# rlorenzo/facet

Measured on NVIDIA B200. Metric: images/sec, higher is better.
Workload: dtype fp16

## Files before the change

facet_b200/csrc/attention_tc.cu:

```cuda
#include <cuda_bf16.h>

#include "common.cuh"
#include "kernels.h"
#include "tc_common.cuh"

namespace fb {

namespace {

constexpr int kTok = 257, kW = 1024, kD = 64;
constexpr int kThreadsAttn = 512;
constexpr float kScaleLog2 = 0.125f * 1.4426950408889634f;

constexpr int kOffQ = 0;
constexpr int kOffK = 32768;
constexpr int kOffV = 65536;
constexpr int kOffX = 98304;
constexpr int kWgBytes = 98304 + 8192;
constexpr int kSmemAttn = 2 * kWgBytes + 1024;

struct XArea {
    uint32_t q256h[32], k256h[32];
    float v256[64];
    float cls_p[264];
    float cls_red[16];
    float cls_o[64];
    float s256[2][128];
    float xmax[2][128];
    float xsum[2][128];
    uint64_t bar_qk, bar_v, bar_s, bar_pv;
};


__device__ __forceinline__ const uint4* sw_chunk(const uint8_t* tile, int r, int c) {
    return reinterpret_cast<const uint4*>(tile + r * 128 + ((c ^ (r & 7)) << 4));
}

template <bool F16>
__device__ __forceinline__ float mac2(uint32_t a, uint32_t b, float acc) {
    if (F16) {
        asm("{.reg .b16 al, ah, bl, bh;\n\t"
            "mov.b32 {al, ah}, %1;\n\t"
            "mov.b32 {bl, bh}, %2;\n\t"
            "fma.rn.f32.f16 %0, al, bl, %0;\n\t"
            "fma.rn.f32.f16 %0, ah, bh, %0;}"
            : "+f"(acc) : "r"(a), "r"(b));
        return acc;
    }
    acc = fmaf(tc::lo16<false>(a), tc::lo16<false>(b), acc);
    return fmaf(tc::hi16<false>(a), tc::hi16<false>(b), acc);
}
template <bool F16>
__device__ __forceinline__ void axpy2(float p, uint32_t p16, uint32_t v, float& a0, float& a1) {
    if (F16) {
        asm("{.reg .b16 pl, ph, vl, vh;\n\t"
            "mov.b32 {pl, ph}, %2;\n\t"
            "mov.b32 {vl, vh}, %3;\n\t"
            "fma.rn.f32.f16 %0, pl, vl, %0;\n\t"
            "fma.rn.f32.f16 %1, pl, vh, %1;}"
            : "+f"(a0), "+f"(a1) : "r"(p16), "r"(v));
        return;
    }
    a0 = fmaf(p, tc::lo16<false>(v), a0);
    a1 = fmaf(p, tc::hi16<false>(v), a1);
}

template <bool F16>
__device__ __forceinline__ float dot64_row(const uint8_t* tile, int r, const uint32_t* vec) {
    float acc = 0.f;
#pragma unroll
    for (int c = 0; c < 8; ++c) {
        const uint4 w = *sw_chunk(tile, r, c);
        const uint4 v = *reinterpret_cast<const uint4*>(vec + 4 * c);
        acc = mac2<F16>(w.x, v.x, acc);
        acc = mac2<F16>(w.y, v.y, acc);
        acc = mac2<F16>(w.z, v.z, acc);
        acc = mac2<F16>(w.w, v.w, acc);
    }
    return acc;
}

__device__ __forceinline__ uint64_t make_desc_mn_sw128(uint32_t smem_addr) {
    const uint32_t lo = ((smem_addr >> 4) & 0x3FFFu) | (64u << 16);
    const uint32_t hi = 64u | (1u << 14) | (2u << 29);
    return ((uint64_t)hi << 32) | lo;
}

__device__ __forceinline__ void umma_bf16_ts(uint32_t tmem_d, uint32_t tmem_a, uint64_t desc_b, uint32_t idesc, uint32_t accumulate) {
    asm volatile(
        "{\n\t.reg .pred p;\n\tsetp.ne.b32 p, %4, 0;\n\t"
        "tcgen05.mma.cta_group::1.kind::f16 [%0], [%1], %2, %3, p;\n\t}"
        ::"r"(tmem_d), "r"(tmem_a), "l"(desc_b), "r"(idesc), "r"(accumulate) : "memory");
}
__device__ __forceinline__ void tmem_st_32x16(uint32_t taddr, const uint32_t (&v)[16]) {
    asm volatile(
        "tcgen05.st.sync.aligned.32x32b.x16.b32 [%0], {%1,%2,%3,%4,%5,%6,%7,%8,%9,%10,%11,%12,%13,%14,%15,%16};"
        ::"r"(taddr), "r"(v[0]), "r"(v[1]), "r"(v[2]), "r"(v[3]), "r"(v[4]), "r"(v[5]), "r"(v[6]), "r"(v[7]), "r"(v[8]),
          "r"(v[9]), "r"(v[10]), "r"(v[11]), "r"(v[12]), "r"(v[13]), "r"(v[14]), "r"(v[15]) : "memory");
}
__device__ __forceinline__ void tmem_st_wait() { asm volatile("tcgen05.wait::st.sync.aligned;" ::: "memory"); }
__device__ __forceinline__ float ex2_fast(float x) {
    float y;
    asm("ex2.approx.ftz.f32 %0, %1;" : "=f"(y) : "f"(x));
    return y;
}
__device__ __forceinline__ void wg_sync(int wg) { asm volatile("bar.sync %0, 256;" ::"r"(wg + 1) : "memory"); }

template <bool F16>
__global__ void __launch_bounds__(kThreadsAttn, 1)
attention_tc_kernel(const __grid_constant__ CUtensorMap tmap_qkv, const uint16_t* __restrict__ qkv,
                    uint16_t* __restrict__ out, int n_pairs) {
    extern __shared__ uint8_t smem_raw[];
    __shared__ uint32_t tmem_slot;
    uint8_t* smem0 = smem_raw + ((1024u - ((uint32_t)__cvta_generic_to_shared(smem_raw) & 1023u)) & 1023u);
    const int tid = threadIdx.x, warp = tid >> 5, lane = tid & 31;
    const int wg = warp >> 3;
    const int wt = tid & 255;
    const int row = wt & 127;
    const int half = wt >> 7;
    uint8_t* smem = smem0 + wg * kWgBytes;
    XArea* X = reinterpret_cast<XArea*>(smem + kOffX);

    if (wt == 0) {
        tc::mbar_init(&X->bar_qk, 1);
        tc::mbar_init(&X->bar_v, 1);
        tc::mbar_init(&X->bar_s, 1);
        tc::mbar_init(&X->bar_pv, 1);
        tc::mbar_fence_init();
        tc::fence_proxy_async();
        if (tid == 0) tc::tma_prefetch_desc(&tmap_qkv);
    }
    if (warp == 0) tc::tmem_alloc(&tmem_slot, 512);
    tc::tc_fence_before();
    __syncthreads();
    tc::tc_fence_after();
    const uint32_t tmem = tmem_slot + wg * 256;
    const uint32_t lane_base = (uint32_t)(32 * (warp & 3)) << 16;
    const uint32_t t_s = tmem + lane_base + half * 128;
    const uint32_t t_p = tmem + lane_base + half * 128;
    const uint32_t t_o = tmem + lane_base + 64 + half * 32;
    const uint32_t idesc_s = tc::make_idesc16<F16>(128, 256);
    const uint32_t idesc_o = tc::make_idesc16<F16>(128, 64, 0, 1);

    const int first = blockIdx.x * 2 + wg, stride = gridDim.x * 2;
    auto issue_qk = [&](int pair) {
        const int b = pair >> 4, h = pair & 15, r0 = b * kTok;
        tc::mbar_expect_tx(&X->bar_qk, 4 * 16384);
        tc::tma_load_2d(&tmap_qkv, &X->bar_qk, smem + kOffQ, h * kD, r0);
        tc::tma_load_2d(&tmap_qkv, &X->bar_qk, smem + kOffQ + 16384, h * kD, r0 + 128);
        tc::tma_load_2d(&tmap_qkv, &X->bar_qk, smem + kOffK, kW + h * kD, r0);
        tc::tma_load_2d(&tmap_qkv, &X->bar_qk, smem + kOffK + 16384, kW + h * kD, r0 + 128);
    };
    auto issue_v = [&](int pair) {
        const int b = pair >> 4, h = pair & 15, r0 = b * kTok;
        tc::mbar_expect_tx(&X->bar_v, 2 * 16384);
        tc::tma_load_2d(&tmap_qkv, &X->bar_v, smem + kOffV, 2 * kW + h * kD, r0);
        tc::tma_load_2d(&tmap_qkv, &X->bar_v, smem + kOffV + 16384, 2 * kW + h * kD, r0 + 128);
    };
    if (wt == 0 && first < n_pairs) {
        issue_qk(first);
        issue_v(first);
    }

    auto load256 = [&](int pair) -> uint32_t {
        const int b = pair >> 4, h = pair & 15;
        return __ldg(reinterpret_cast<const uint32_t*>(qkv + ((size_t)b * kTok + 256) * (3 * kW) + (wt >> 5) * kW + h * kD + (wt & 31) * 2));
    };
    uint32_t pre256 = 0;
    if (wt < 96 && first < n_pairs) pre256 = load256(first);
    const int w8 = warp & 7;

    uint32_t ph_load = 0, ph_s = 0, ph_pv = 0;
    for (int pair = first; pair < n_pairs; pair += stride) {
        const int b = pair >> 4, h = pair & 15;
        const size_t tok0 = (size_t)b * kTok;
        const int next = pair + stride;
        if (wt < 96) {
            const int which = wt >> 5, i2 = wt & 31;
            if (which == 0) X->q256h[i2] = pre256;
            else if (which == 1) X->k256h[i2] = pre256;
            else {
                X->v256[2 * i2] = tc::lo16<F16>(pre256);
                X->v256[2 * i2 + 1] = tc::hi16<F16>(pre256);
            }
        }
        wg_sync(wg);
        tc::mbar_wait(&X->bar_qk, ph_load);
        if (wt == 0) {
            const uint64_t dk = tc::make_desc_k_sw128(tc::smem_u32(smem + kOffK));
            const uint64_t dq = tc::make_desc_k_sw128(tc::smem_u32(smem + kOffQ));
#pragma unroll
            for (int k = 0; k < 4; ++k) tc::umma_bf16(tmem, dq + 2 * k, dk + 2 * k, idesc_s, k != 0);
            tc::umma_commit(&X->bar_s);
        }
        X->s256[half][row] = dot64_row<F16>(smem + kOffQ + half * 16384, row, X->k256h);

#pragma unroll 1
        for (int t = 0; t < 2; ++t) {
            tc::mbar_wait(&X->bar_s, ph_s);
            ph_s ^= 1;
            tc::tc_fence_after();
            if (t == 1 && wt == 0 && next < n_pairs) issue_qk(next);
            float mx;
            {
                uint32_t va[32], vb[32];
                float m0 = half == 0 ? X->s256[t][row] : -INFINITY, m1 = -INFINITY, m2 = -INFINITY, m3 = -INFINITY;
                tc::tmem_ld_32x32(t_s, va);
#pragma unroll 1
                for (int c = 0; c < 4; c += 2) {
                    tc::tmem_ld_wait();
                    tc::tmem_ld_32x32(t_s + (c + 1) * 32, vb);
#pragma unroll
                    for (int j = 0; j < 32; j += 4) {
                        m0 = fmaxf(m0, __uint_as_float(va[j]));
                        m1 = fmaxf(m1, __uint_as_float(va[j + 1]));
                        m2 = fmaxf(m2, __uint_as_float(va[j + 2]));
                        m3 = fmaxf(m3, __uint_as_float(va[j + 3]));
                    }
                    tc::tmem_ld_wait();
                    if (c + 2 < 4) tc::tmem_ld_32x32(t_s + (c + 2) * 32, va);
#pragma unroll
                    for (int j = 0; j < 32; j += 4) {
                        m0 = fmaxf(m0, __uint_as_float(vb[j]));
                        m1 = fmaxf(m1, __uint_as_float(vb[j + 1]));
                        m2 = fmaxf(m2, __uint_as_float(vb[j + 2]));
                        m3 = fmaxf(m3, __uint_as_float(vb[j + 3]));
                    }
                }
                mx = fmaxf(fmaxf(m0, m1), fmaxf(m2, m3));
            }
            X->xmax[half][row] = mx;
            wg_sync(wg);
            mx = fmaxf(X->xmax[0][row], X->xmax[1][row]);
            const float s256 = X->s256[t][row];
            const float mxs = mx * kScaleLog2;
            const float p_last = ex2_fast(fmaf(s256, kScaleLog2, -mxs));
            float sum0 = half == 0 ? p_last : 0.f, sum1 = 0.f;
            {
                uint32_t va[32], vb[32];
                auto emit = [&](const uint32_t (&v)[32], int c) {
                    uint32_t pk[16];
#pragma unroll
                    for (int j = 0; j < 16; ++j) {
                        const float x0 = fmaf(__uint_as_float(v[2 * j]), kScaleLog2, -mxs);
                        const float x1 = fmaf(__uint_as_float(v[2 * j + 1]), kScaleLog2, -mxs);
                        const float p0 = ex2_fast(x0), p1 = ex2_fast(x1);
                        sum0 += p0;
                        sum1 += p1;
                        pk[j] = tc::pack16<F16>(p0, p1);
                    }
                    tmem_st_32x16(t_p + c * 16, pk);
                };
                tc::tmem_ld_32x32(t_s, va);
#pragma unroll 1
                for (int c = 0; c < 4; c += 2) {
                    tc::tmem_ld_wait();
                    tc::tmem_ld_32x32(t_s + (c + 1) * 32, vb);
                    emit(va, c);
                    tc::tmem_ld_wait();
                    if (c + 2 < 4) tc::tmem_ld_32x32(t_s + (c + 2) * 32, va);
                    emit(vb, c + 1);
                }
            }
            X->xsum[half][row] = sum0 + sum1;
            tmem_st_wait();
            tc::tc_fence_before();
            wg_sync(wg);
            const float inv_l = 1.0f / (X->xsum[0][row] + X->xsum[1][row]);
            if (t == 0) tc::mbar_wait(&X->bar_v, ph_load);
            if (wt == 0) {
                tc::tc_fence_after();
                const uint32_t vbase = tc::smem_u32(smem + kOffV);
#pragma unroll
                for (int i = 0; i < 16; ++i)
                    umma_bf16_ts(tmem + 64, tmem + (i < 8 ? 8 * i : 128 + 8 * (i - 8)), make_desc_mn_sw128(vbase + i * 2048), idesc_o, i != 0);
                tc::umma_commit(&X->bar_pv);
            }
            if (t == 0) {
                const float sa = dot64_row<F16>(smem + kOffK, wt, X->q256h);
                float s_last = -INFINITY;
                if (wt == 0) {
                    s_last = 0.f;
#pragma unroll
                    for (int d = 0; d < 32; ++d) s_last = mac2<F16>(X->q256h[d], X->k256h[d], s_last);
                }
                float cm = fmaxf(sa, s_last);
#pragma unroll
                for (int o = 16; o > 0; o >>= 1) cm = fmaxf(cm, __shfl_xor_sync(0xffffffffu, cm, o));
                if (lane == 0) X->cls_red[w8] = cm;
                wg_sync(wg);
                cm = fmaxf(fmaxf(fmaxf(X->cls_red[0], X->cls_red[1]), fmaxf(X->cls_red[2], X->cls_red[3])),
                           fmaxf(fmaxf(X->cls_red[4], X->cls_red[5]), fmaxf(X->cls_red[6], X->cls_red[7])));
                const float pa = ex2_fast((sa - cm) * kScaleLog2);
                X->cls_p[wt] = pa;
                float sum = pa;
                if (wt == 0) {
                    const float pl = ex2_fast((s_last - cm) * kScaleLog2);
                    X->cls_p[256] = pl;
                    sum += pl;
                }
#pragma unroll
                for (int o = 16; o > 0; o >>= 1) sum += __shfl_xor_sync(0xffffffffu, sum, o);
                if (lane == 0) X->cls_red[8 + w8] = sum;
            } else {
                if (wt < 96 && next < n_pairs) pre256 = load256(next);
                float a8[8];
#pragma unroll
                for (int k = 0; k < 8; ++k) a8[k] = 0.f;
#pragma unroll
                for (int i = 0; i < 8; ++i) {
                    const int key = lane + 32 * i;
                    const uint4 q = *sw_chunk(smem + kOffV, key, w8);
                    const float pj = X->cls_p[key];
                    const uint32_t p16 = F16 ? tc::pack_f16(pj, pj) : 0u;
                    axpy2<F16>(pj, p16, q.x, a8[0], a8[1]);
                    axpy2<F16>(pj, p16, q.y, a8[2], a8[3]);
                    axpy2<F16>(pj, p16, q.z, a8[4], a8[5]);
                    axpy2<F16>(pj, p16, q.w, a8[6], a8[7]);
                }
                float b4[4], b2[2];
                const bool u16 = (lane & 16) != 0, u8 = (lane & 8) != 0, u4 = (lane & 4) != 0;
#pragma unroll
                for (int k = 0; k < 4; ++k) {
                    const float send = u16 ? a8[k] : a8[k + 4];
                    const float keep = u16 ? a8[k + 4] : a8[k];
                    b4[k] = keep + __shfl_xor_sync(0xffffffffu, send, 16);
                }
#pragma unroll
                for (int k = 0; k < 2; ++k) {
                    const float send = u8 ? b4[k] : b4[k + 2];
                    const float keep = u8 ? b4[k + 2] : b4[k];
                    b2[k] = keep + __shfl_xor_sync(0xffffffffu, send, 8);
                }
                float tot1 = (u4 ? b2[1] : b2[0]) + __shfl_xor_sync(0xffffffffu, u4 ? b2[0] : b2[1], 4);
                tot1 += __shfl_xor_sync(0xffffffffu, tot1, 2);
                tot1 += __shfl_xor_sync(0xffffffffu, tot1, 1);
                if ((lane & 3) == 0) X->cls_o[8 * w8 + (u16 ? 4 : 0) + (u8 ? 2 : 0) + (u4 ? 1 : 0)] = tot1;
            }
            tc::mbar_wait(&X->bar_pv, ph_pv);
            ph_pv ^= 1;
            tc::tc_fence_after();
            {
                uint32_t v0[32];
                tc::tmem_ld_32x32(t_o, v0);
                tc::tmem_ld_wait();
                tc::tc_fence_before();
                wg_sync(wg);
                if (t == 0 && wt == 0) {
                    tc::tc_fence_after();
                    const uint64_t dk = tc::make_desc_k_sw128(tc::smem_u32(smem + kOffK));
                    const uint64_t dq = tc::make_desc_k_sw128(tc::smem_u32(smem + kOffQ + 16384));
#pragma unroll
                    for (int k = 0; k < 4; ++k) tc::umma_bf16(tmem, dq + 2 * k, dk + 2 * k, idesc_s, k != 0);
                    tc::umma_commit(&X->bar_s);
                }
                if (t == 1) {
                    if (wt == 0 && next < n_pairs) issue_v(next);
                    if (wt < 64) {
                        const float tot = ((X->cls_red[8] + X->cls_red[9]) + (X->cls_red[10] + X->cls_red[11])) +
                                          ((X->cls_red[12] + X->cls_red[13]) + (X->cls_red[14] + X->cls_red[15]));
                        const float o = X->cls_o[wt] + X->cls_p[256] * X->v256[wt];
                        out[(tok0 + 256) * kW + h * kD + wt] = (uint16_t)(tc::pack16<F16>(o / tot, 0.f) & 0xffffu);
                    }
                }
                uint4* dst = reinterpret_cast<uint4*>(out + (tok0 + t * 128 + row) * kW + h * kD + half * 32);
#pragma unroll
                for (int q = 0; q < 4; ++q) {
                    float o[8];
#pragma unroll
                    for (int j = 0; j < 8; ++j) {
                        const int dcol = 8 * q + j;
                        o[j] = (__uint_as_float(v0[dcol]) + p_last * X->v256[half * 32 + dcol]) * inv_l;
                    }
                    dst[q] = make_uint4(tc::pack16<F16>(o[0], o[1]), tc::pack16<F16>(o[2], o[3]), tc::pack16<F16>(o[4], o[5]),
                                        tc::pack16<F16>(o[6], o[7]));
                }
            }
        }
        ph_load ^= 1;
        wg_sync(wg);
    }
    tc::tc_fence_before();
    __syncthreads();
    tc::tc_fence_after();
    if (warp == 0) tc::tmem_dealloc(tmem_slot, 512);
}

}

int launch_attention_tc(const void* d_qkv, int batch, void* d_out, int f16, cudaStream_t stream) {
    FB_REQUIRE(d_qkv && d_out && batch >= 1, "fb_vit_attention: bad arguments");
    CUtensorMap tm;
    int rc = make_tmap_bf16_2d(&tm, d_qkv, (uint64_t)batch * kTok, 3 * kW, 3 * kW, 128, 64);
    if (rc) return rc;
    static PerDeviceFlag attr_set;
    if (!attr_set.get()) {
        FB_CUDA_OK(cudaFuncSetAttribute(attention_tc_kernel<false>, cudaFuncAttributeMaxDynamicSharedMemorySize, kSmemAttn));
        FB_CUDA_OK(cudaFuncSetAttribute(attention_tc_kernel<true>, cudaFuncAttributeMaxDynamicSharedMemorySize, kSmemAttn));
        attr_set.set();
    }
    const int n_pairs = batch * 16;
    int grid = (n_pairs + 1) / 2;
    if (grid > sm_count()) grid = sm_count();
    if (f16) attention_tc_kernel<true><<<grid, kThreadsAttn, kSmemAttn, stream>>>(tm, reinterpret_cast<const uint16_t*>(d_qkv),
                                                                              reinterpret_cast<uint16_t*>(d_out), n_pairs);
    else attention_tc_kernel<false><<<grid, kThreadsAttn, kSmemAttn, stream>>>(tm, reinterpret_cast<const uint16_t*>(d_qkv),
                                                                            reinterpret_cast<uint16_t*>(d_out), n_pairs);
    FB_CUDA_OK(cudaGetLastError());
    return 0;
}

}
```

facet_b200/csrc/tc_common.cuh:

```cuda
#pragma once
#include <cuda.h>
#include <cuda_bf16.h>
#include <cuda_fp16.h>
#include <cuda_runtime.h>
#include <stdint.h>

namespace fb {
namespace tc {

__device__ __forceinline__ uint32_t smem_u32(const void* p) { return (uint32_t)__cvta_generic_to_shared(p); }

__device__ __forceinline__ bool elect_one() {
    uint32_t pred = 0;
    asm volatile(
        "{\n\t.reg .pred P;\n\telect.sync _|P, 0xffffffff;\n\tselp.b32 %0, 1, 0, P;\n\t}"
        : "=r"(pred));
    return pred != 0;
}

__device__ __forceinline__ void mbar_init(uint64_t* bar, uint32_t count) {
    asm volatile("mbarrier.init.shared::cta.b64 [%0], %1;" ::"r"(smem_u32(bar)), "r"(count));
}
__device__ __forceinline__ void mbar_fence_init() {
    asm volatile("fence.mbarrier_init.release.cluster;" ::: "memory");
}
__device__ __forceinline__ void fence_proxy_async() {
    asm volatile("fence.proxy.async.shared::cta;" ::: "memory");
}
__device__ __forceinline__ void mbar_expect_tx(uint64_t* bar, uint32_t bytes) {
    asm volatile("mbarrier.arrive.expect_tx.shared::cta.b64 _, [%0], %1;" ::"r"(smem_u32(bar)), "r"(bytes) : "memory");
}
__device__ __forceinline__ void mbar_arrive(uint64_t* bar) {
    asm volatile("mbarrier.arrive.shared::cta.b64 _, [%0];" ::"r"(smem_u32(bar)) : "memory");
}
__device__ __forceinline__ void mbar_wait(uint64_t* bar, uint32_t parity) {
    const uint32_t addr = smem_u32(bar);
    asm volatile(
        "{\n\t"
        ".reg .pred P1;\n\t"
        "WAIT_%=:\n\t"
        "mbarrier.try_wait.parity.shared::cta.b64 P1, [%0], %1;\n\t"
        "@P1 bra DONE_%=;\n\t"
        "bra WAIT_%=;\n\t"
        "DONE_%=:\n\t"
        "}" ::"r"(addr), "r"(parity) : "memory");
}

__device__ __forceinline__ void tma_prefetch_desc(const CUtensorMap* m) {
    asm volatile("prefetch.tensormap [%0];" ::"l"(reinterpret_cast<uint64_t>(m)) : "memory");
}
__device__ __forceinline__ void tma_load_2d(const CUtensorMap* m, uint64_t* bar, void* smem_dst, int c0, int c1) {
    asm volatile(
        "cp.async.bulk.tensor.2d.shared::cluster.global.mbarrier::complete_tx::bytes [%0], [%1, {%3, %4}], [%2];"
        ::"r"(smem_u32(smem_dst)), "l"(reinterpret_cast<uint64_t>(m)), "r"(smem_u32(bar)), "r"(c0), "r"(c1)
        : "memory");
}

__device__ __forceinline__ void tma_load_2d_multicast(const CUtensorMap* m, uint64_t* bar, void* smem_dst, int c0, int c1,
                                                      uint16_t cta_mask) {
    asm volatile(
        "cp.async.bulk.tensor.2d.shared::cluster.global.mbarrier::complete_tx::bytes.multicast::cluster [%0], [%1, {%3, %4}], [%2], %5;"
        ::"r"(smem_u32(smem_dst)), "l"(reinterpret_cast<uint64_t>(m)), "r"(smem_u32(bar)), "r"(c0), "r"(c1), "h"(cta_mask)
        : "memory");
}
__device__ __forceinline__ uint32_t mapa_u32(uint32_t local, uint32_t rank) {
    uint32_t r;
    asm volatile("mapa.shared::cluster.u32 %0, %1, %2;" : "=r"(r) : "r"(local), "r"(rank));
    return r;
}
__device__ __forceinline__ void mbar_expect_tx_cluster(uint32_t cluster_addr, uint32_t bytes) {
    asm volatile("mbarrier.arrive.expect_tx.shared::cluster.b64 _, [%0], %1;" ::"r"(cluster_addr), "r"(bytes) : "memory");
}
__device__ __forceinline__ void mbar_arrive_cluster(uint32_t cluster_addr) {
    asm volatile("mbarrier.arrive.shared::cluster.b64 _, [%0];" ::"r"(cluster_addr) : "memory");
}
__device__ __forceinline__ void tma_load_2d_pair(const CUtensorMap* m, uint32_t bar_cluster_addr, void* smem_dst, int c0, int c1) {
    asm volatile(
        "cp.async.bulk.tensor.2d.cta_group::2.shared::cluster.global.mbarrier::complete_tx::bytes [%0], [%1, {%3, %4}], [%2];"
        ::"r"(smem_u32(smem_dst)), "l"(reinterpret_cast<uint64_t>(m)), "r"(bar_cluster_addr), "r"(c0), "r"(c1)
        : "memory");
}
__device__ __forceinline__ void tmem_alloc_pair(uint32_t* smem_dst, uint32_t cols) {
    asm volatile("tcgen05.alloc.cta_group::2.sync.aligned.shared::cta.b32 [%0], %1;" ::"r"(smem_u32(smem_dst)), "r"(cols) : "memory");
    asm volatile("tcgen05.relinquish_alloc_permit.cta_group::2.sync.aligned;" ::: "memory");
}
__device__ __forceinline__ void tmem_dealloc_pair(uint32_t taddr, uint32_t cols) {
    asm volatile("tcgen05.dealloc.cta_group::2.sync.aligned.b32 %0, %1;" ::"r"(taddr), "r"(cols) : "memory");
}
__device__ __forceinline__ void umma_bf16_pair(uint32_t tmem_d, uint64_t desc_a, uint64_t desc_b, uint32_t idesc, uint32_t accumulate) {
    asm volatile(
        "{\n\t.reg .pred p;\n\tsetp.ne.b32 p, %4, 0;\n\t"
        "tcgen05.mma.cta_group::2.kind::f16 [%0], %1, %2, %3, p;\n\t}"
        ::"r"(tmem_d), "l"(desc_a), "l"(desc_b), "r"(idesc), "r"(accumulate) : "memory");
}
__device__ __forceinline__ void umma_commit_pair(uint64_t* bar, uint16_t cta_mask) {
    asm volatile("tcgen05.commit.cta_group::2.mbarrier::arrive::one.shared::cluster.multicast::cluster.b64 [%0], %1;"
                 ::"r"(smem_u32(bar)), "h"(cta_mask) : "memory");
}
__device__ __forceinline__ uint32_t cluster_ctarank() {
    uint32_t r;
    asm volatile("mov.u32 %0, %%cluster_ctarank;" : "=r"(r));
    return r;
}
__device__ __forceinline__ void cluster_sync_all() {
    asm volatile("barrier.cluster.arrive.release.aligned;\n\tbarrier.cluster.wait.acquire.aligned;" ::: "memory");
}

__device__ __forceinline__ void tmem_alloc(uint32_t* smem_dst, uint32_t cols) {
    asm volatile("tcgen05.alloc.cta_group::1.sync.aligned.shared::cta.b32 [%0], %1;" ::"r"(smem_u32(smem_dst)), "r"(cols) : "memory");
    asm volatile("tcgen05.relinquish_alloc_permit.cta_group::1.sync.aligned;" ::: "memory");
}
__device__ __forceinline__ void tmem_dealloc(uint32_t taddr, uint32_t cols) {
    asm volatile("tcgen05.dealloc.cta_group::1.sync.aligned.b32 %0, %1;" ::"r"(taddr), "r"(cols) : "memory");
}
__device__ __forceinline__ void tc_fence_before() { asm volatile("tcgen05.fence::before_thread_sync;" ::: "memory"); }
__device__ __forceinline__ void tc_fence_after() { asm volatile("tcgen05.fence::after_thread_sync;" ::: "memory"); }

__device__ __forceinline__ void umma_bf16(uint32_t tmem_d, uint64_t desc_a, uint64_t desc_b, uint32_t idesc, uint32_t accumulate) {
    asm volatile(
        "{\n\t.reg .pred p;\n\tsetp.ne.b32 p, %4, 0;\n\t"
        "tcgen05.mma.cta_group::1.kind::f16 [%0], %1, %2, %3, p;\n\t}"
        ::"r"(tmem_d), "l"(desc_a), "l"(desc_b), "r"(idesc), "r"(accumulate) : "memory");
}
__device__ __forceinline__ void umma_commit(uint64_t* bar) {
    asm volatile("tcgen05.commit.cta_group::1.mbarrier::arrive::one.shared::cluster.b64 [%0];" ::"r"(smem_u32(bar)) : "memory");
}

__device__ __forceinline__ void umma_commit_multicast(uint64_t* bar, uint16_t cta_mask) {
    asm volatile("tcgen05.commit.cta_group::1.mbarrier::arrive::one.shared::cluster.multicast::cluster.b64 [%0], %1;"
                 ::"r"(smem_u32(bar)), "h"(cta_mask) : "memory");
}

__host__ __device__ constexpr uint32_t make_idesc_bf16(int m, int n, int a_mn_major = 0, int b_mn_major = 0) {
    return (1u << 4) | (1u << 7) | (1u << 10) | ((uint32_t)a_mn_major << 15) | ((uint32_t)b_mn_major << 16) |
           ((uint32_t)(n >> 3) << 17) | ((uint32_t)(m >> 4) << 24);
}
__host__ __device__ constexpr uint32_t make_idesc_f16(int m, int n, int a_mn_major = 0, int b_mn_major = 0) {
    return (1u << 4) | ((uint32_t)a_mn_major << 15) | ((uint32_t)b_mn_major << 16) |
           ((uint32_t)(n >> 3) << 17) | ((uint32_t)(m >> 4) << 24);
}
template <bool F16>
__host__ __device__ constexpr uint32_t make_idesc16(int m, int n, int a_mn_major = 0, int b_mn_major = 0) {
    return F16 ? make_idesc_f16(m, n, a_mn_major, b_mn_major) : make_idesc_bf16(m, n, a_mn_major, b_mn_major);
}

__device__ __forceinline__ uint64_t make_desc_k_sw128(uint32_t smem_addr) {
    const uint32_t lo = ((smem_addr >> 4) & 0x3FFFu) | (1u << 16);
    const uint32_t hi = 64u | (1u << 14) | (2u << 29);
    return ((uint64_t)hi << 32) | lo;
}

__device__ __forceinline__ void tmem_ld_32x32(uint32_t taddr, uint32_t (&v)[32]) {
    asm volatile(
        "tcgen05.ld.sync.aligned.32x32b.x32.b32 "
        "{%0,%1,%2,%3,%4,%5,%6,%7,%8,%9,%10,%11,%12,%13,%14,%15,%16,%17,%18,%19,%20,%21,%22,%23,%24,%25,%26,%27,%28,%29,%30,%31}, [%32];"
        : "=r"(v[0]), "=r"(v[1]), "=r"(v[2]), "=r"(v[3]), "=r"(v[4]), "=r"(v[5]), "=r"(v[6]), "=r"(v[7]), "=r"(v[8]),
          "=r"(v[9]), "=r"(v[10]), "=r"(v[11]), "=r"(v[12]), "=r"(v[13]), "=r"(v[14]), "=r"(v[15]), "=r"(v[16]),
          "=r"(v[17]), "=r"(v[18]), "=r"(v[19]), "=r"(v[20]), "=r"(v[21]), "=r"(v[22]), "=r"(v[23]), "=r"(v[24]),
          "=r"(v[25]), "=r"(v[26]), "=r"(v[27]), "=r"(v[28]), "=r"(v[29]), "=r"(v[30]), "=r"(v[31])
        : "r"(taddr) : "memory");
}
__device__ __forceinline__ void tmem_ld_wait() { asm volatile("tcgen05.wait::ld.sync.aligned;" ::: "memory"); }

__device__ __forceinline__ uint32_t pack_bf16(float a, float b) {
    __nv_bfloat162 v = __floats2bfloat162_rn(a, b);
    return *reinterpret_cast<uint32_t*>(&v);
}
__device__ __forceinline__ uint32_t pack_f16(float a, float b) {
    __half2 v = __floats2half2_rn(a, b);
    return *reinterpret_cast<uint32_t*>(&v);
}
template <bool F16>
__device__ __forceinline__ uint32_t pack16(float a, float b) { return F16 ? pack_f16(a, b) : pack_bf16(a, b); }
template <bool F16>
__device__ __forceinline__ float lo16(uint32_t w) {
    if (F16) return __half2float(__ushort_as_half((unsigned short)(w & 0xffffu)));
    return __uint_as_float(w << 16);
}
template <bool F16>
__device__ __forceinline__ float hi16(uint32_t w) {
    if (F16) return __half2float(__ushort_as_half((unsigned short)(w >> 16)));
    return __uint_as_float(w & 0xffff0000u);
}

}

int make_tmap_bf16_2d(CUtensorMap* out, const void* base, uint64_t rows, uint64_t cols, uint64_t row_stride_elems,
                      uint32_t box_rows, uint32_t box_cols);

}
```

Measured before the change: 4183.

## Warp-specialize attention kernel with double-buffered TMA pipeline and TMA output stores

Restructures the ViT attention kernel from two independent 256-thread workgroups into a warp-specialized design: one TMA producer warp, one MMA issuer warp, eight softmax warps and two warps dedicated to the CLS token row. Inputs are double-buffered with full/empty mbarriers, and the score matrix is split into four 128-key blocks whose partial softmaxes are merged with rescaling. Outputs are staged in shared memory and written with TMA stores, and the dot product uses four independent accumulators. The aim is to overlap loads, MMA and softmax across pairs, at the cost of more complex synchronization and one pair per CTA instead of two.

```diff
diff --git a/facet_b200/csrc/attention_tc.cu b/facet_b200/csrc/attention_tc.cu
--- a/facet_b200/csrc/attention_tc.cu
+++ b/facet_b200/csrc/attention_tc.cu
@@ -9,28 +9,29 @@
 namespace {
 
 constexpr int kTok = 257, kW = 1024, kD = 64;
-constexpr int kThreadsAttn = 512;
+constexpr int kThreadsAttn = 384;
 constexpr float kScaleLog2 = 0.125f * 1.4426950408889634f;
 
 constexpr int kOffQ = 0;
 constexpr int kOffK = 32768;
 constexpr int kOffV = 65536;
-constexpr int kOffX = 98304;
-constexpr int kWgBytes = 98304 + 8192;
-constexpr int kSmemAttn = 2 * kWgBytes + 1024;
-
-struct XArea {
-    uint32_t q256h[32], k256h[32];
-    float v256[64];
+constexpr int kBufBytes = 98304;
+constexpr int kTileBytes = 16384;
+
+struct Tok256 {
+    uint32_t q[32], k[32];
+    float v[64];
+};
+struct Ctl {
+    Tok256 tok[2];
     float cls_p[264];
-    float cls_red[16];
+    float cls_red[4];
     float cls_o[64];
-    float s256[2][128];
-    float xmax[2][128];
-    float xsum[2][128];
-    uint64_t bar_qk, bar_v, bar_s, bar_pv;
+    uint64_t full[2], empty[2];
+    uint64_t s_ready[4], p_ready[4], o_ready[4], blk_free[4];
 };
-
+constexpr int kSmemAttn = 2 * kBufBytes + (int)sizeof(Ctl) + 1024;
+constexpr uint32_t kEmptyArrivals = 256 + 64 + 1;
 
 __device__ __forceinline__ const uint4* sw_chunk(const uint8_t* tile, int r, int c) {
     return reinterpret_cast<const uint4*>(tile + r * 128 + ((c ^ (r & 7)) << 4));
@@ -67,17 +68,17 @@
 
 template <bool F16>
 __device__ __forceinline__ float dot64_row(const uint8_t* tile, int r, const uint32_t* vec) {
-    float acc = 0.f;
+    float a0 = 0.f, a1 = 0.f, a2 = 0.f, a3 = 0.f;
 #pragma unroll
     for (int c = 0; c < 8; ++c) {
         const uint4 w = *sw_chunk(tile, r, c);
         const uint4 v = *reinterpret_cast<const uint4*>(vec + 4 * c);
-        acc = mac2<F16>(w.x, v.x, acc);
-        acc = mac2<F16>(w.y, v.y, acc);
-        acc = mac2<F16>(w.z, v.z, acc);
-        acc = mac2<F16>(w.w, v.w, acc);
-    }
-    return acc;
+        a0 = mac2<F16>(w.x, v.x, a0);
+        a1 = mac2<F16>(w.y, v.y, a1);
+        a2 = mac2<F16>(w.z, v.z, a2);
+        a3 = mac2<F16>(w.w, v.w, a3);
+    }
+    return (a0 + a1) + (a2 + a3);
 }
 
 __device__ __forceinline__ uint64_t make_desc_mn_sw128(uint32_t smem_addr) {
@@ -104,286 +105,278 @@
     asm("ex2.approx.ftz.f32 %0, %1;" : "=f"(y) : "f"(x));
     return y;
 }
-__device__ __forceinline__ void wg_sync(int wg) { asm volatile("bar.sync %0, 256;" ::"r"(wg + 1) : "memory"); }
+__device__ __forceinline__ void cls_sync() { asm volatile("bar.sync 1, 64;" ::: "memory"); }
 
 template <bool F16>
 __global__ void __launch_bounds__(kThreadsAttn, 1)
-attention_tc_kernel(const __grid_constant__ CUtensorMap tmap_qkv, const uint16_t* __restrict__ qkv,
-                    uint16_t* __restrict__ out, int n_pairs) {
+attention_tc_kernel(const __grid_constant__ CUtensorMap tmap_qkv, const __grid_constant__ CUtensorMap tmap_out,
+                    const uint16_t* __restrict__ qkv, uint16_t* __restrict__ out, int n_pairs) {
     extern __shared__ uint8_t smem_raw[];
     __shared__ uint32_t tmem_slot;
-    uint8_t* smem0 = smem_raw + ((1024u - ((uint32_t)__cvta_generic_to_shared(smem_raw) & 1023u)) & 1023u);
+    uint8_t* smem = smem_raw + ((1024u - ((uint32_t)__cvta_generic_to_shared(smem_raw) & 1023u)) & 1023u);
+    Ctl* C = reinterpret_cast<Ctl*>(smem + 2 * kBufBytes);
     const int tid = threadIdx.x, warp = tid >> 5, lane = tid & 31;
-    const int wg = warp >> 3;
-    const int wt = tid & 255;
-    const int row = wt & 127;
-    const int half = wt >> 7;
-    uint8_t* smem = smem0 + wg * kWgBytes;
-    XArea* X = reinterpret_cast<XArea*>(smem + kOffX);
-
-    if (wt == 0) {
-        tc::mbar_init(&X->bar_qk, 1);
-        tc::mbar_init(&X->bar_v, 1);
-        tc::mbar_init(&X->bar_s, 1);
-        tc::mbar_init(&X->bar_pv, 1);
+
+    if (tid == 0) {
+        for (int b = 0; b < 2; ++b) {
+            tc::mbar_init(&C->full[b], 2);
+            tc::mbar_init(&C->empty[b], kEmptyArrivals);
+        }
+        for (int k = 0; k < 4; ++k) {
+            tc::mbar_init(&C->s_ready[k], 1);
+            tc::mbar_init(&C->p_ready[k], 128);
+            tc::mbar_init(&C->o_ready[k], 1);
+            tc::mbar_init(&C->blk_free[k], 128);
+        }
         tc::mbar_fence_init();
         tc::fence_proxy_async();
-        if (tid == 0) tc::tma_prefetch_desc(&tmap_qkv);
+        tc::tma_prefetch_desc(&tmap_qkv);
+        tc::tma_prefetch_desc(&tmap_out);
     }
     if (warp == 0) tc::tmem_alloc(&tmem_slot, 512);
     tc::tc_fence_before();
     __syncthreads();
     tc::tc_fence_after();
-    const uint32_t tmem = tmem_slot + wg * 256;
-    const uint32_t lane_base = (uint32_t)(32 * (warp & 3)) << 16;
-    const uint32_t t_s = tmem + lane_base + half * 128;
-    const uint32_t t_p = tmem + lane_base + half * 128;
-    const uint32_t t_o = tmem + lane_base + 64 + half * 32;
-    const uint32_t idesc_s = tc::make_idesc16<F16>(128, 256);
-    const uint32_t idesc_o = tc::make_idesc16<F16>(128, 64, 0, 1);
-
-    const int first = blockIdx.x * 2 + wg, stride = gridDim.x * 2;
-    auto issue_qk = [&](int pair) {
-        const int b = pair >> 4, h = pair & 15, r0 = b * kTok;
-        tc::mbar_expect_tx(&X->bar_qk, 4 * 16384);
-        tc::tma_load_2d(&tmap_qkv, &X->bar_qk, smem + kOffQ, h * kD, r0);
-        tc::tma_load_2d(&tmap_qkv, &X->bar_qk, smem + kOffQ + 16384, h * kD, r0 + 128);
-        tc::tma_load_2d(&tmap_qkv, &X->bar_qk, smem + kOffK, kW + h * kD, r0);
-        tc::tma_load_2d(&tmap_qkv, &X->bar_qk, smem + kOffK + 16384, kW + h * kD, r0 + 128);
-    };
-    auto issue_v = [&](int pair) {
-        const int b = pair >> 4, h = pair & 15, r0 = b * kTok;
-        tc::mbar_expect_tx(&X->bar_v, 2 * 16384);
-        tc::tma_load_2d(&tmap_qkv, &X->bar_v, smem + kOffV, 2 * kW + h * kD, r0);
-        tc::tma_load_2d(&tmap_qkv, &X->bar_v, smem + kOffV + 16384, 2 * kW + h * kD, r0 + 128);
-    };
-    if (wt == 0 && first < n_pairs) {
-        issue_qk(first);
-        issue_v(first);
-    }
-
-    auto load256 = [&](int pair) -> uint32_t {
-        const int b = pair >> 4, h = pair & 15;
-        return __ldg(reinterpret_cast<const uint32_t*>(qkv + ((size_t)b * kTok + 256) * (3 * kW) + (wt >> 5) * kW + h * kD + (wt & 31) * 2));
-    };
-    uint32_t pre256 = 0;
-    if (wt < 96 && first < n_pairs) pre256 = load256(first);
-    const int w8 = warp & 7;
-
-    uint32_t ph_load = 0, ph_s = 0, ph_pv = 0;
-    for (int pair = first; pair < n_pairs; pair += stride) {
-        const int b = pair >> 4, h = pair & 15;
-        const size_t tok0 = (size_t)b * kTok;
-        const int next = pair + stride;
-        if (wt < 96) {
-            const int which = wt >> 5, i2 = wt & 31;
-            if (which == 0) X->q256h[i2] = pre256;
-            else if (which == 1) X->k256h[i2] = pre256;
-            else {
-                X->v256[2 * i2] = tc::lo16<F16>(pre256);
-                X->v256[2 * i2 + 1] = tc::hi16<F16>(pre256);
-            }
-        }
-        wg_sync(wg);
-        tc::mbar_wait(&X->bar_qk, ph_load);
-        if (wt == 0) {
-            const uint64_t dk = tc::make_desc_k_sw128(tc::smem_u32(smem + kOffK));
-            const uint64_t dq = tc::make_desc_k_sw128(tc::smem_u32(smem + kOffQ));
-#pragma unroll
-            for (int k = 0; k < 4; ++k) tc::umma_bf16(tmem, dq + 2 * k, dk + 2 * k, idesc_s, k != 0);
-            tc::umma_commit(&X->bar_s);
-        }
-        X->s256[half][row] = dot64_row<F16>(smem + kOffQ + half * 16384, row, X->k256h);
-
-#pragma unroll 1
-        for (int t = 0; t < 2; ++t) {
-            tc::mbar_wait(&X->bar_s, ph_s);
-            ph_s ^= 1;
+    const uint32_t tmem = tmem_slot;
+
+    if (warp < 8) {
+        const int t = warp >> 2;
+        const int row = 32 * (warp & 3) + lane;
+        const uint32_t t_row = tmem + ((uint32_t)(32 * (warp & 3)) << 16);
+        auto block_softmax = [&](int blk, uint32_t ph, float& m_out, float& l_out) {
+            const uint32_t ta = t_row + 128 * blk;
+            tc::mbar_wait(&C->s_ready[blk], ph);
             tc::tc_fence_after();
-            if (t == 1 && wt == 0 && next < n_pairs) issue_qk(next);
-            float mx;
-            {
-                uint32_t va[32], vb[32];
-                float m0 = half == 0 ? X->s256[t][row] : -INFINITY, m1 = -INFINITY, m2 = -INFINITY, m3 = -INFINITY;
-                tc::tmem_ld_32x32(t_s, va);
-#pragma unroll 1
-                for (int c = 0; c < 4; c += 2) {
-                    tc::tmem_ld_wait();
-                    tc::tmem_ld_32x32(t_s + (c + 1) * 32, vb);
-#pragma unroll
-                    for (int j = 0; j < 32; j += 4) {
-                        m0 = fmaxf(m0, __uint_as_float(va[j]));
-                        m1 = fmaxf(m1, __uint_as_float(va[j + 1]));
-                        m2 = fmaxf(m2, __uint_as_float(va[j + 2]));
-                        m3 = fmaxf(m3, __uint_as_float(va[j + 3]));
-                    }
-                    tc::tmem_ld_wait();
-                    if (c + 2 < 4) tc::tmem_ld_32x32(t_s + (c + 2) * 32, va);
-#pragma unroll
-                    for (int j = 0; j < 32; j += 4) {
-                        m0 = fmaxf(m0, __uint_as_float(vb[j]));
-                        m1 = fmaxf(m1, __uint_as_float(vb[j + 1]));
-                        m2 = fmaxf(m2, __uint_as_float(vb[j + 2]));
-                        m3 = fmaxf(m3, __uint_as_float(vb[j + 3]));
-                    }
-                }
-                mx = fmaxf(fmaxf(m0, m1), fmaxf(m2, m3));
-            }
-            X->xmax[half][row] = mx;
-            wg_sync(wg);
-            mx = fmaxf(X->xmax[0][row], X->xmax[1][row]);
-            const float s256 = X->s256[t][row];
+            uint32_t v[4][32];
+#pragma unroll
+            for (int c = 0; c < 4; ++c) tc::tmem_ld_32x32(ta + 32 * c, v[c]);
+            tc::tmem_ld_wait();
+            float m0 = -INFINITY, m1 = -INFINITY, m2 = -INFINITY, m3 = -INFINITY;
+#pragma unroll
+            for (int c = 0; c < 4; ++c)
+#pragma unroll
+                for (int j = 0; j < 32; j += 4) {
+                    m0 = fmaxf(m0, __uint_as_float(v[c][j]));
+                    m1 = fmaxf(m1, __uint_as_float(v[c][j + 1]));
+                    m2 = fmaxf(m2, __uint_as_float(v[c][j + 2]));
+                    m3 = fmaxf(m3, __uint_as_float(v[c][j + 3]));
+                }
+            const float mx = fmaxf(fmaxf(m0, m1), fmaxf(m2, m3));
             const float mxs = mx * kScaleLog2;
-            const float p_last = ex2_fast(fmaf(s256, kScaleLog2, -mxs));
-            float sum0 = half == 0 ? p_last : 0.f, sum1 = 0.f;
-            {
-                uint32_t va[32], vb[32];
-                auto emit = [&](const uint32_t (&v)[32], int c) {
-                    uint32_t pk[16];
-#pragma unroll
-                    for (int j = 0; j < 16; ++j) {
-                        const float x0 = fmaf(__uint_as_float(v[2 * j]), kScaleLog2, -mxs);
-                        const float x1 = fmaf(__uint_as_float(v[2 * j + 1]), kScaleLog2, -mxs);
-                        const float p0 = ex2_fast(x0), p1 = ex2_fast(x1);
-                        sum0 += p0;
-                        sum1 += p1;
-                        pk[j] = tc::pack16<F16>(p0, p1);
-                    }
-                    tmem_st_32x16(t_p + c * 16, pk);
-                };
-                tc::tmem_ld_32x32(t_s, va);
-#pragma unroll 1
-                for (int c = 0; c < 4; c += 2) {
-                    tc::tmem_ld_wait();
-                    tc::tmem_ld_32x32(t_s + (c + 1) * 32, vb);
-                    emit(va, c);
-                    tc::tmem_ld_wait();
-                    if (c + 2 < 4) tc::tmem_ld_32x32(t_s + (c + 2) * 32, va);
-                    emit(vb, c + 1);
-                }
-            }
-            X->xsum[half][row] = sum0 + sum1;
+            float sum0 = 0.f, sum1 = 0.f;
+#pragma unroll
+            for (int c = 0; c < 4; ++c) {
+                uint32_t pk[16];
+#pragma unroll
+                for (int j = 0; j < 16; ++j) {
+                    const float p0 = ex2_fast(fmaf(__uint_as_float(v[c][2 * j]), kScaleLog2, -mxs));
+                    const float p1 = ex2_fast(fmaf(__uint_as_float(v[c][2 * j + 1]), kScaleLog2, -mxs));
+                    sum0 += p0;
+                    sum1 += p1;
+                    pk[j] = tc::pack16<F16>(p0, p1);
+                }
+                tmem_st_32x16(ta + 16 * c, pk);
+            }
             tmem_st_wait();
             tc::tc_fence_before();
-            wg_sync(wg);
-            const float inv_l = 1.0f / (X->xsum[0][row] + X->xsum[1][row]);
-            if (t == 0) tc::mbar_wait(&X->bar_v, ph_load);
-            if (wt == 0) {
+            tc::mbar_arrive(&C->p_ready[blk]);
+            m_out = mx;
+            l_out = sum0 + sum1;
+        };
+        int it = 0;
+        for (int pair = blockIdx.x; pair < n_pairs; pair += gridDim.x, ++it) {
+            const int b = it & 1;
+            const uint32_t ph = it & 1;
+            uint8_t* buf = smem + b * kBufBytes;
+            const Tok256& tk = C->tok[b];
+            tc::mbar_wait(&C->full[b], (it >> 1) & 1);
+            float m0, l0, m1, l1;
+            block_softmax(2 * t, ph, m0, l0);
+            block_softmax(2 * t + 1, ph, m1, l1);
+            uint32_t o0[2][32];
+            tc::mbar_wait(&C->o_ready[2 * t], ph);
+            tc::tc_fence_after();
+            tc::tmem_ld_32x32(t_row + 128 * (2 * t) + 64, o0[0]);
+            tc::tmem_ld_32x32(t_row + 128 * (2 * t) + 96, o0[1]);
+            tc::tmem_ld_wait();
+            tc::tc_fence_before();
+            tc::mbar_arrive(&C->blk_free[2 * t]);
+            const float s_last = dot64_row<F16>(buf + kOffQ + t * kTileBytes, row, tk.k);
+            const float m = fmaxf(fmaxf(m0, m1), s_last);
+            const float a0 = ex2_fast((m0 - m) * kScaleLog2), a1 = ex2_fast((m1 - m) * kScaleLog2);
+            const float a2 = ex2_fast((s_last - m) * kScaleLog2);
+            const float inv_l = 1.0f / (fmaf(a0, l0, a1 * l1) + a2);
+            const float c0 = a0 * inv_l, c1 = a1 * inv_l, cl = a2 * inv_l;
+
+            tc::mbar_wait(&C->o_ready[2 * t + 1], ph);
+            tc::tc_fence_after();
+            uint8_t* stage = buf + kOffQ + t * kTileBytes;
+#pragma unroll
+            for (int c = 0; c < 2; ++c) {
+                uint32_t u1[32];
+                tc::tmem_ld_32x32(t_row + 128 * (2 * t + 1) + 64 + 32 * c, u1);
+                tc::tmem_ld_wait();
+                if (c == 1) {
+                    tc::tc_fence_before();
+                    tc::mbar_arrive(&C->blk_free[2 * t + 1]);
+                }
+#pragma unroll
+                for (int q = 0; q < 4; ++q) {
+                    uint32_t w[4];
+#pragma unroll
+                    for (int k = 0; k < 4; ++k) {
+                        const int d = 8 * q + 2 * k;
+                        const float2 vv = *reinterpret_cast<const float2*>(&tk.v[32 * c + d]);
+                        const float o0a = fmaf(__uint_as_float(u1[d]), c1, fmaf(__uint_as_float(o0[c][d]), c0, cl * vv.x));
+                        const float o0b = fmaf(__uint_as_float(u1[d + 1]), c1, fmaf(__uint_as_float(o0[c][d + 1]), c0, cl * vv.y));
+                        w[k] = tc::pack16<F16>(o0a, o0b);
+                    }
+                    *reinterpret_cast<uint4*>(stage + row * 128 + (((4 * c + q) ^ (row & 7)) << 4)) = make_uint4(w[0], w[1], w[2], w[3]);
+                }
+            }
+            tc::fence_proxy_async();
+            if (t == 0) asm volatile("bar.sync 2, 128;" ::: "memory");
+            else asm volatile("bar.sync 3, 128;" ::: "memory");
+            if (row == 0) {
+                tc::tma_store_2d(&tmap_out, stage, (pair & 15) * kD, (pair >> 4) * kTok + t * 128);
+                tc::bulk_commit_group();
+                tc::bulk_wait_group_read0();
+            }
+            tc::mbar_arrive(&C->empty[b]);
+        }
+        if (row == 0) tc::bulk_wait_group0();
+    } else if (warp == 8) {
+        int it = 0;
+        for (int pair = blockIdx.x; pair < n_pairs; pair += gridDim.x, ++it) {
+            const int b = it & 1;
+            if (it >= 2) tc::mbar_wait(&C->empty[b], ((it >> 1) - 1) & 1);
+            const int img = pair >> 4, h = pair & 15, r0 = img * kTok;
+            uint8_t* buf = smem + b * kBufBytes;
+            if (lane == 0) {
+                tc::mbar_expect_tx(&C->full[b], 6 * kTileBytes);
+                tc::tma_load_2d(&tmap_qkv, &C->full[b], buf + kOffQ, h * kD, r0);
+                tc::tma_load_2d(&tmap_qkv, &C->full[b], buf + kOffQ + kTileBytes, h * kD, r0 + 128);
+                tc::tma_load_2d(&tmap_qkv, &C->full[b], buf + kOffK, kW + h * kD, r0);
+                tc::tma_load_2d(&tmap_qkv, &C->full[b], buf + kOffK + kTileBytes, kW + h * kD, r0 + 128);
+                tc::tma_load_2d(&tmap_qkv, &C->full[b], buf + kOffV, 2 * kW + h * kD, r0);
+                tc::tma_load_2d(&tmap_qkv, &C->full[b], buf + kOffV + kTileBytes, 2 * kW + h * kD, r0 + 128);
+            }
+            const uint32_t* src = reinterpret_cast<const uint32_t*>(qkv + ((size_t)r0 + 256) * (3 * kW) + h * kD) + lane;
+            const uint32_t q = __ldg(src), k = __ldg(src + kW / 2), v = __ldg(src + kW);
+            C->tok[b].q[lane] = q;
+            C->tok[b].k[lane] = k;
+            C->tok[b].v[2 * lane] = tc::lo16<F16>(v);
+            C->tok[b].v[2 * lane + 1] = tc::hi16<F16>(v);
+            __syncwarp();
+            if (lane == 0) tc::mbar_arrive(&C->full[b]);
+        }
+    } else if (warp == 9) {
+        if (lane == 0) {
+            const uint32_t idesc_s = tc::make_idesc16<F16>(128, 128);
+            const uint32_t idesc_o = tc::make_idesc16<F16>(128, 64, 0, 1);
+            int it = 0;
+            for (int pair = blockIdx.x; pair < n_pairs; pair += gridDim.x, ++it) {
+                const int b = it & 1;
+                const uint32_t ph = it & 1;
+                const uint8_t* buf = smem + b * kBufBytes;
+                tc::mbar_wait(&C->full[b], (it >> 1) & 1);
                 tc::tc_fence_after();
-                const uint32_t vbase = tc::smem_u32(smem + kOffV);
-#pragma unroll
-                for (int i = 0; i < 16; ++i)
-                    umma_bf16_ts(tmem + 64, tmem + (i < 8 ? 8 * i : 128 + 8 * (i - 8)), make_desc_mn_sw128(vbase + i * 2048), idesc_o, i != 0);
-                tc::umma_commit(&X->bar_pv);
-            }
-            if (t == 0) {
-                const float sa = dot64_row<F16>(smem + kOffK, wt, X->q256h);
-                float s_last = -INFINITY;
-                if (wt == 0) {
-                    s_last = 0.f;
-#pragma unroll
-                    for (int d = 0; d < 32; ++d) s_last = mac2<F16>(X->q256h[d], X->k256h[d], s_last);
-                }
-                float cm = fmaxf(sa, s_last);
-#pragma unroll
-                for (int o = 16; o > 0; o >>= 1) cm = fmaxf(cm, __shfl_xor_sync(0xffffffffu, cm, o));
-                if (lane == 0) X->cls_red[w8] = cm;
-                wg_sync(wg);
-                cm = fmaxf(fmaxf(fmaxf(X->cls_red[0], X->cls_red[1]), fmaxf(X->cls_red[2], X->cls_red[3])),
-                           fmaxf(fmaxf(X->cls_red[4], X->cls_red[5]), fmaxf(X->cls_red[6], X->cls_red[7])));
-                const float pa = ex2_fast((sa - cm) * kScaleLog2);
-                X->cls_p[wt] = pa;
-                float sum = pa;
-                if (wt == 0) {
-                    const float pl = ex2_fast((s_last - cm) * kScaleLog2);
-                    X->cls_p[256] = pl;
-                    sum += pl;
-                }
-#pragma unroll
-                for (int o = 16; o > 0; o >>= 1) sum += __shfl_xor_sync(0xffffffffu, sum, o);
-                if (lane == 0) X->cls_red[8 + w8] = sum;
-            } else {
-                if (wt < 96 && next < n_pairs) pre256 = load256(next);
-                float a8[8];
-#pragma unroll
-                for (int k = 0; k < 8; ++k) a8[k] = 0.f;
-#pragma unroll
-                for (int i = 0; i < 8; ++i) {
-                    const int key = lane + 32 * i;
-                    const uint4 q = *sw_chunk(smem + kOffV, key, w8);
-                    const float pj = X->cls_p[key];
-                    const uint32_t p16 = F16 ? tc::pack_f16(pj, pj) : 0u;
-                    axpy2<F16>(pj, p16, q.x, a8[0], a8[1]);
-                    axpy2<F16>(pj, p16, q.y, a8[2], a8[3]);
-                    axpy2<F16>(pj, p16, q.z, a8[4], a8[5]);
-                    axpy2<F16>(pj, p16, q.w, a8[6], a8[7]);
-                }
-                float b4[4], b2[2];
-                const bool u16 = (lane & 16) != 0, u8 = (lane & 8) != 0, u4 = (lane & 4) != 0;
-#pragma unroll
-                for (int k = 0; k < 4; ++k) {
-                    const float send = u16 ? a8[k] : a8[k + 4];
-                    const float keep = u16 ? a8[k + 4] : a8[k];
-                    b4[k] = keep + __shfl_xor_sync(0xffffffffu, send, 16);
-                }
-#pragma unroll
-                for (int k = 0; k < 2; ++k) {
-                    const float send = u8 ? b4[k] : b4[k + 2];
-                    const float keep = u8 ? b4[k + 2] : b4[k];
-                    b2[k] = keep + __shfl_xor_sync(0xffffffffu, send, 8);
-                }
-                float tot1 = (u4 ? b2[1] : b2[0]) + __shfl_xor_sync(0xffffffffu, u4 ? b2[0] : b2[1], 4);
-                tot1 += __shfl_xor_sync(0xffffffffu, tot1, 2);
-                tot1 += __shfl_xor_sync(0xffffffffu, tot1, 1);
-                if ((lane & 3) == 0) X->cls_o[8 * w8 + (u16 ? 4 : 0) + (u8 ? 2 : 0) + (u4 ? 1 : 0)] = tot1;
-            }
-            tc::mbar_wait(&X->bar_pv, ph_pv);
-            ph_pv ^= 1;
-            tc::tc_fence_after();
-            {
-                uint32_t v0[32];
-                tc::tmem_ld_32x32(t_o, v0);
-                tc::tmem_ld_wait();
-                tc::tc_fence_before();
-                wg_sync(wg);
-                if (t == 0 && wt == 0) {
+#pragma unroll 1
+                for (int i = 0; i < 4; ++i) {
+                    const int t = i & 1, h = i >> 1, blk = 2 * t + h;
+                    if (it > 0) {
+                        tc::mbar_wait(&C->blk_free[blk], ph ^ 1);
+                        tc::tc_fence_after();
+                    }
+                    const uint64_t dq = tc::make_desc_k_sw128(tc::smem_u32(buf + kOffQ + t * kTileBytes));
+                    const uint64_t dk = tc::make_desc_k_sw128(tc::smem_u32(buf + kOffK + h * kTileBytes));
+#pragma unroll
+                    for (int k = 0; k < 4; ++k) tc::umma_bf16(tmem + 128 * blk, dq + 2 * k, dk + 2 * k, idesc_s, k != 0);
+                    tc::umma_commit(&C->s_ready[blk]);
+                }
+#pragma unroll 1
+                for (int i = 0; i < 4; ++i) {
+                    const int t = i & 1, h = i >> 1, blk = 2 * t + h;
+                    tc::mbar_wait(&C->p_ready[blk], ph);
                     tc::tc_fence_after();
-                    const uint64_t dk = tc::make_desc_k_sw128(tc::smem_u32(smem + kOffK));
-                    const uint64_t dq = tc::make_desc_k_sw128(tc::smem_u32(smem + kOffQ + 16384));
-#pragma unroll
-                    for (int k = 0; k < 4; ++k) tc::umma_bf16(tmem, dq + 2 * k, dk + 2 * k, idesc_s, k != 0);
-                    tc::umma_commit(&X->bar_s);
-                }
-                if (t == 1) {
-                    if (wt == 0 && next < n_pairs) issue_v(next);
-                    if (wt < 64) {
-                        const float tot = ((X->cls_red[8] + X->cls_red[9]) + (X->cls_red[10] + X->cls_red[11])) +
-                                          ((X->cls_red[12] + X->cls_red[13]) + (X->cls_red[14] + X->cls_red[15]));
-                        const float o = X->cls_o[wt] + X->cls_p[256] * X->v256[wt];
-                        out[(tok0 + 256) * kW + h * kD + wt] = (uint16_t)(tc::pack16<F16>(o / tot, 0.f) & 0xffffu);
-                    }
-                }
-                uint4* dst = reinterpret_cast<uint4*>(out + (tok0 + t * 128 + row) * kW + h * kD + half * 32);
-#pragma unroll
-                for (int q = 0; q < 4; ++q) {
-                    float o[8];
-#pragma unroll
-                    for (int j = 0; j < 8; ++j) {
-                        const int dcol = 8 * q + j;
-                        o[j] = (__uint_as_float(v0[dcol]) + p_last * X->v256[half * 32 + dcol]) * inv_l;
-                    }
-                    dst[q] = make_uint4(tc::pack16<F16>(o[0], o[1]), tc::pack16<F16>(o[2], o[3]), tc::pack16<F16>(o[4], o[5]),
-                                        tc::pack16<F16>(o[6], o[7]));
-                }
-            }
-        }
-        ph_load ^= 1;
-        wg_sync(wg);
+                    const uint32_t vbase = tc::smem_u32(buf + kOffV + h * kTileBytes);
+#pragma unroll
+                    for (int k = 0; k < 8; ++k)
+                        umma_bf16_ts(tmem + 128 * blk + 64, tmem + 128 * blk + 8 * k, make_desc_mn_sw128(vbase + k * 2048), idesc_o, k != 0);
+                    tc::umma_commit(&C->o_ready[blk]);
+                }
+                tc::umma_commit(&C->empty[b]);
+            }
+        }
+        __syncwarp();
+    } else if (warp >= 10) {
+        const int ct = tid - 320, cw = warp - 10;
+        int it = 0;
+        for (int pair = blockIdx.x; pair < n_pairs; pair += gridDim.x, ++it) {
+            const int b = it & 1;
+            const uint8_t* buf = smem + b * kBufBytes;
+            const Tok256& tk = C->tok[b];
+            tc::mbar_wait(&C->full[b], (it >> 1) & 1);
+            float s[4];
+#pragma unroll
+            for (int k = 0; k < 4; ++k) s[k] = dot64_row<F16>(buf + kOffK, ct + 64 * k, tk.q);
+            float s_last = -INFINITY;
+            if (ct == 0) {
+                s_last = 0.f;
+#pragma unroll
+                for (int d = 0; d < 32; ++d) s_last = mac2<F16>(tk.q[d], tk.k[d], s_last);
+            }
+            float cm = fmaxf(fmaxf(fmaxf(s[0], s[1]), fmaxf(s[2], s[3])), s_last);
+#pragma unroll
+            for (int o = 16; o > 0; o >>= 1) cm = fmaxf(cm, __shfl_xor_sync(0xffffffffu, cm, o));
+            if (lane == 0) C->cls_red[cw] = cm;
+            cls_sync();
+            cm = fmaxf(C->cls_red[0], C->cls_red[1]);
+            float sum = 0.f;
+#pragma unroll
+            for (int k = 0; k < 4; ++k) {
+                const float p = ex2_fast((s[k] - cm) * kScaleLog2);
+                C->cls_p[ct + 64 * k] = p;
+                sum += p;
+            }
+            if (ct == 0) {
+                const float p = ex2_fast((s_last - cm) * kScaleLog2);
+                C->cls_p[256] = p;
+                sum += p;
+            }
+#pragma unroll
+            for (int o = 16; o > 0; o >>= 1) sum += __shfl_xor_sync(0xffffffffu, sum, o);
+            if (lane == 0) C->cls_red[2 + cw] = sum;
+            cls_sync();
+            const uint8_t* vt = buf + kOffV;
+            float a0 = 0.f, a1 = 0.f;
+#pragma unroll 8
+            for (int j = 0; j < 128; ++j) {
+                const int key = 128 * cw + j;
+                const uint32_t w = *reinterpret_cast<const uint32_t*>(vt + key * 128 + ((((lane >> 2) ^ (key & 7)) << 4) | ((lane & 3) << 2)));
+                const float pj = C->cls_p[key];
+                axpy2<F16>(pj, F16 ? tc::pack_f16(pj, pj) : 0u, w, a0, a1);
+            }
+            if (cw == 1) {
+                C->cls_o[2 * lane] = a0;
+                C->cls_o[2 * lane + 1] = a1;
+            }
+            cls_sync();
+            if (cw == 0) {
+                const float inv = 1.0f / (C->cls_red[2] + C->cls_red[3]), pl = C->cls_p[256];
+                const float o0 = (a0 + C->cls_o[2 * lane] + pl * tk.v[2 * lane]) * inv;
+                const float o1 = (a1 + C->cls_o[2 * lane + 1] + pl * tk.v[2 * lane + 1]) * inv;
+                const int img = pair >> 4, h = pair & 15;
+                reinterpret_cast<uint32_t*>(out + ((size_t)img * kTok + 256) * kW + h * kD)[lane] = tc::pack16<F16>(o0, o1);
+            }
+            tc::mbar_arrive(&C->empty[b]);
+            cls_sync();
+        }
     }
     tc::tc_fence_before();
     __syncthreads();
     tc::tc_fence_after();
-    if (warp == 0) tc::tmem_dealloc(tmem_slot, 512);
+    if (warp == 0) tc::tmem_dealloc(tmem, 512);
 }
 
 }
@@ -392,6 +385,9 @@
     FB_REQUIRE(d_qkv && d_out && batch >= 1, "fb_vit_attention: bad arguments");
     CUtensorMap tm;
     int rc = make_tmap_bf16_2d(&tm, d_qkv, (uint64_t)batch * kTok, 3 * kW, 3 * kW, 128, 64);
+    if (rc) return rc;
+    CUtensorMap tm_out;
+    rc = make_tmap_bf16_2d(&tm_out, d_out, (uint64_t)batch * kTok, kW, kW, 128, 64);
     if (rc) return rc;
     static PerDeviceFlag attr_set;
     if (!attr_set.get()) {
@@ -400,11 +396,11 @@
         attr_set.set();
     }
     const int n_pairs = batch * 16;
-    int grid = (n_pairs + 1) / 2;
+    int grid = n_pairs;
     if (grid > sm_count()) grid = sm_count();
-    if (f16) attention_tc_kernel<true><<<grid, kThreadsAttn, kSmemAttn, stream>>>(tm, reinterpret_cast<const uint16_t*>(d_qkv),
+    if (f16) attention_tc_kernel<true><<<grid, kThreadsAttn, kSmemAttn, stream>>>(tm, tm_out, reinterpret_cast<const uint16_t*>(d_qkv),
                                                                               reinterpret_cast<uint16_t*>(d_out), n_pairs);
-    else attention_tc_kernel<false><<<grid, kThreadsAttn, kSmemAttn, stream>>>(tm, reinterpret_cast<const uint16_t*>(d_qkv),
+    else attention_tc_kernel<false><<<grid, kThreadsAttn, kSmemAttn, stream>>>(tm, tm_out, reinterpret_cast<const uint16_t*>(d_qkv),
                                                                             reinterpret_cast<uint16_t*>(d_out), n_pairs);
     FB_CUDA_OK(cudaGetLastError());
     return 0;
diff --git a/facet_b200/csrc/tc_common.cuh b/facet_b200/csrc/tc_common.cuh
--- a/facet_b200/csrc/tc_common.cuh
+++ b/facet_b200/csrc/tc_common.cuh
@@ -55,6 +55,14 @@
         ::"r"(smem_u32(smem_dst)), "l"(reinterpret_cast<uint64_t>(m)), "r"(smem_u32(bar)), "r"(c0), "r"(c1)
         : "memory");
 }
+
+__device__ __forceinline__ void tma_store_2d(const CUtensorMap* m, const void* smem_src, int c0, int c1) {
+    asm volatile("cp.async.bulk.tensor.2d.global.shared::cta.bulk_group [%0, {%2, %3}], [%1];"
+                 ::"l"(reinterpret_cast<uint64_t>(m)), "r"(smem_u32(smem_src)), "r"(c0), "r"(c1) : "memory");
+}
+__device__ __forceinline__ void bulk_commit_group() { asm volatile("cp.async.bulk.commit_group;" ::: "memory"); }
+__device__ __forceinline__ void bulk_wait_group_read0() { asm volatile("cp.async.bulk.wait_group.read 0;" ::: "memory"); }
+__device__ __forceinline__ void bulk_wait_group0() { asm volatile("cp.async.bulk.wait_group 0;" ::: "memory"); }
 
 __device__ __forceinline__ void tma_load_2d_multicast(const CUtensorMap* m, uint64_t* bar, void* smem_dst, int c0, int c1,
                                                       uint16_t cta_mask) {
```

After: 4210, median of 6. No clear change (+0.7%).
